# GiannisPikoulis/dsml-thesis

Measured on AMD Instinct MI355X. Metric: DDIM denoise steps/sec (64×64×4 latent, 256² face) at 1/2/4/8 GPUs, higher is better.
Workload: dtype f32; 1 GPU; face_reenactment emotion-conditioned LDM (AffectNet config), DDIM-200 schedule, 16 samples/GPU, 64x64x4 latent, CFG off, eta 0, random-init weights; batch_per_gpu=16, global_batch=16, ddim_steps=200, hipgraph=True

## Files before the change

### dsml_thesis_amd/csrc/winograd.hip

```cpp
#include "ldmk_common.h"
#include "ldmk_split.h"

namespace ldmk {

__global__ __launch_bounds__(256) void wino_input_kernel(const float* __restrict__ x0, int c0, const float* __restrict__ x1,
                                                         int c1, const float* __restrict__ coef, int silu, int H, int W,
                                                         long long tiles, float* __restrict__ V) {
  const int C = c0 + c1, c4n = C >> 2;
  const int tw = W >> 1, th = H >> 1;
  const long long total = tiles * c4n;
  for (long long idx = (long long)blockIdx.x * blockDim.x + threadIdx.x; idx < total; idx += (long long)gridDim.x * blockDim.x) {
    const long long t = idx / c4n;
    const int c = (int)(idx - t * c4n) * 4;
    const int tx = (int)(t % tw);
    const long long t2 = t / tw;
    const int ty = (int)(t2 % th), n = (int)(t2 / th);
    const float* src = c < c0 ? x0 + (long long)n * H * W * c0 + c : x1 + (long long)n * H * W * c1 + (c - c0);
    const int cs = c < c0 ? c0 : c1;
    float4 sc = make_float4(1.f, 1.f, 1.f, 1.f), sh = make_float4(0.f, 0.f, 0.f, 0.f);
    if (coef) {
      const float* cf = coef + ((long long)n * 2) * C + c;
      sc = *reinterpret_cast<const float4*>(cf);
      sh = *reinterpret_cast<const float4*>(cf + C);
    }
// ... 88 lines not shown
    const int cs = c < c0 ? c0 : c1;
    float4 sc[2] = {make_float4(1.f, 1.f, 1.f, 1.f), make_float4(1.f, 1.f, 1.f, 1.f)};
    float4 sh[2] = {make_float4(0.f, 0.f, 0.f, 0.f), make_float4(0.f, 0.f, 0.f, 0.f)};
    if (coef) {
      const float* cf = coef + ((long long)n * 2) * C + c;
      sc[0] = *reinterpret_cast<const float4*>(cf); sc[1] = *reinterpret_cast<const float4*>(cf + 4);
      sh[0] = *reinterpret_cast<const float4*>(cf + C); sh[1] = *reinterpret_cast<const float4*>(cf + C + 4);
    }
#pragma unroll
    for (int i = 0; i < 4; ++i) {
      const int y = 2 * ty - 1 + i;
#pragma unroll
      for (int j = 0; j < 4; ++j) {
        const int x = 2 * tx - 1 + j;
        const bool in = y >= 0 && y < H && x >= 0 && x < W;
#pragma unroll
        for (int e = 0; e < 2; ++e) {
          float4 v = make_float4(0.f, 0.f, 0.f, 0.f);
          if (in) {
            v = *reinterpret_cast<const float4*>(src + ((long long)y * W + x) * cs + 4 * e);
            if (coef) { v.x = fmaf(v.x, sc[e].x, sh[e].x); v.y = fmaf(v.y, sc[e].y, sh[e].y); v.z = fmaf(v.z, sc[e].z, sh[e].z); v.w = fmaf(v.w, sc[e].w, sh[e].w); }
            if (silu) { v.x = silu_f(v.x); v.y = silu_f(v.y); v.z = silu_f(v.z); v.w = silu_f(v.w); }
          }
          d[i][j][e] = v;
        }
      }
    }
  } else {
#pragma unroll
    for (int i = 0; i < 4; ++i)
#pragma unroll
      for (int j = 0; j < 4; ++j) d[i][j][0] = d[i][j][1] = make_float4(0.f, 0.f, 0.f, 0.f);
  }
  auto sub = [](float4 a, float4 b) { return make_float4(a.x - b.x, a.y - b.y, a.z - b.z, a.w - b.w); };
  auto add = [](float4 a, float4 b) { return make_float4(a.x + b.x, a.y + b.y, a.z + b.z, a.w + b.w); };
  unsigned char* dst = V + ((long long)blockIdx.x * Kb + slab) * (PL * 1024) + lane * 16;
#pragma unroll
  for (int i = 0; i < 4; ++i) {
    float4 rr[4][2];
#pragma unroll
    for (int e = 0; e < 2; ++e)
#pragma unroll
      for (int j = 0; j < 4; ++j) {
        rr[j][e] = i == 0 ? sub(d[0][j][e], d[2][j][e]) : i == 1 ? add(d[1][j][e], d[2][j][e]) : i == 2 ? sub(d[2][j][e], d[1][j][e])
                                                                                                          : sub(d[1][j][e], d[3][j][e]);
      }
    wino_store_ps<PL>(dst + (4 * i + 0) * plane_bytes, sub(rr[0][0], rr[2][0]), sub(rr[0][1], rr[2][1]), range_flag);
    wino_store_ps<PL>(dst + (4 * i + 1) * plane_bytes, add(rr[1][0], rr[2][0]), add(rr[1][1], rr[2][1]), range_flag);
    wino_store_ps<PL>(dst + (4 * i + 2) * plane_bytes, sub(rr[2][0], rr[1][0]), sub(rr[2][1], rr[1][1]), range_flag);
    wino_store_ps<PL>(dst + (4 * i + 3) * plane_bytes, sub(rr[1][0], rr[3][0]), sub(rr[1][1], rr[3][1]), range_flag);
  }
}

constexpr int WINO_MAX_CHUNKS = 8;
__global__ __launch_bounds__(256) void wino_output_kernel(const float* __restrict__ Mb, const float* __restrict__ bias,
                                                          const float* __restrict__ bvec, int bvec_ld,
                                                          const float* __restrict__ res, float* __restrict__ out,
                                                          float* __restrict__ stats, int H, int W, int N, int R,
                                                          long long tiles) {
  const int tw = W >> 1, th = H >> 1;
  const int bands = th / R;
  const int n = blockIdx.x / bands, band = blockIdx.x - n * bands;
  const long long ps = tiles * N;
  const int nchunks = (2 * R * W) >> 5;
  const int c = blockIdx.y * blockDim.x + threadIdx.x;
  if (c < N) {
    const float add0 = (bias ? bias[c] : 0.f) + (bvec ? bvec[(long long)n * bvec_ld + c] : 0.f);
    float shift[WINO_MAX_CHUNKS], sm[WINO_MAX_CHUNKS], sq[WINO_MAX_CHUNKS];
    bool have[WINO_MAX_CHUNKS];
#pragma unroll
    for (int k = 0; k < WINO_MAX_CHUNKS; ++k) { shift[k] = 0.f; sm[k] = 0.f; sq[k] = 0.f; have[k] = false; }
    for (int r = 0; r < R; ++r) {
      const int ty = band * R + r;
      for (int tx = 0; tx < tw; ++tx) {
        const long long t = ((long long)n * th + ty) * tw + tx;
        const float* mp = Mb + t * N + c;
        float m[16];
#pragma unroll
        for (int p = 0; p < 16; ++p) m[p] = mp[p * ps];
        float s0[4], s1[4];
#pragma unroll
        for (int j = 0; j < 4; ++j) {
          s0[j] = (m[j] + m[4 + j]) + m[8 + j];
          s1[j] = (m[4 + j] - m[8 + j]) - m[12 + j];
        }
        float y[2][2];
        y[0][0] = (s0[0] + s0[1]) + s0[2];
        y[0][1] = (s0[1] - s0[2]) - s0[3];
        y[1][0] = (s1[0] + s1[1]) + s1[2];
        y[1][1] = (s1[1] - s1[2]) - s1[3];
#pragma unroll
        for (int i = 0; i < 2; ++i)
#pragma unroll
          for (int j = 0; j < 2; ++j) {
            const int yy = 2 * ty + i, xx = 2 * tx + j;
            const long long o = (((long long)n * H + yy) * W + xx) * N + c;
            float v = y[i][j] + add0;
            if (res) v += res[o];
            out[o] = v;
            if (stats) {
              const int k = (((2 * r + i) * W) + xx) >> 5;
#pragma unroll
              for (int q = 0; q < WINO_MAX_CHUNKS; ++q)
                if (q == k) {
                  if (!have[q]) { shift[q] = v; have[q] = true; }
                  const float dv = v - shift[q];
                  sm[q] += dv;
                  sq[q] = fmaf(dv, dv, sq[q]);
                }
            }
          }
      }
    }
    if (stats) {
      const long long chunk0 = ((long long)n * H * W + (long long)band * 2 * R * W) >> 5;
#pragma unroll
      for (int q = 0; q < WINO_MAX_CHUNKS; ++q)
        if (q < nchunks) {
          float* d = stats + ((chunk0 + q) * N + c) * 3;
          d[0] = shift[q]; d[1] = sm[q]; d[2] = sq[q];
        }
    }
  }
}

}

extern "C" long long ldmk_winograd_tiles(int n, int h, int w) { return (long long)n * (h / 2) * (w / 2); }

extern "C" int ldmk_winograd_input(const float* x0, int c0, const float* x1, int c1, const float* coef, int silu, int n, int h,
                                   int w, float* v, void* stream) {
  LDMK_ENTER();
  using namespace ldmk;
  LDMK_REQUIRE(x0 && v && n > 0 && c0 > 0, "ldmk_winograd_input: bad args");
  LDMK_REQUIRE((c1 == 0) == (x1 == nullptr), "ldmk_winograd_input: x1/c1 mismatch");
  LDMK_REQUIRE(h >= 2 && w >= 2 && h % 2 == 0 && w % 2 == 0, "ldmk_winograd_input: H=%d W=%d must be even", h, w);
  LDMK_REQUIRE(c0 % 4 == 0 && c1 % 4 == 0, "ldmk_winograd_input: channel counts must be multiples of 4");
  const long long tiles = ldmk_winograd_tiles(n, h, w);
  const long long total = tiles * ((c0 + c1) / 4);
  long long g = (total + 255) / 256;
  if (g > 16384) g = 16384;
  hipLaunchKernelGGL(wino_input_kernel, dim3((unsigned)g), dim3(256), 0, (hipStream_t)stream, x0, c0, x1, c1, coef, silu, h, w,
                     tiles, v);
  return check_launch("ldmk_winograd_input");
}

extern "C" long long ldmk_ps_bytes(int rows, int k);
extern "C" long long ldmk_ps_bytes_h2(int rows, int k);

static int winograd_input_ps_any(const float* x0, int c0, const float* x1, int c1, const float* coef, int silu, int n, int h, int w, void* v_ps,
                                 int* range_flag, void* stream);

extern "C" int ldmk_winograd_input_ps(const float* x0, int c0, const float* x1, int c1, const float* coef, int silu, int n, int h,
                                      int w, void* v_ps, void* stream) {
  return winograd_input_ps_any(x0, c0, x1, c1, coef, silu, n, h, w, v_ps, nullptr, stream);
}

extern "C" int ldmk_winograd_input_ps_h2(const float* x0, int c0, const float* x1, int c1, const float* coef, int silu, int n, int h,
                                         int w, void* v_ps, int* range_flag, void* stream) {
  LDMK_ENTER();
  LDMK_REQUIRE(range_flag != nullptr, "ldmk_winograd_input_ps_h2: range_flag");
  return winograd_input_ps_any(x0, c0, x1, c1, coef, silu, n, h, w, v_ps, range_flag, stream);
}

static int winograd_input_ps_any(const float* x0, int c0, const float* x1, int c1, const float* coef, int silu, int n, int h, int w, void* v_ps,
                                 int* range_flag, void* stream) {
  LDMK_ENTER();
  using namespace ldmk;
  LDMK_REQUIRE(x0 && v_ps && n > 0 && c0 > 0, "ldmk_winograd_input_ps: bad args");
  LDMK_REQUIRE((c1 == 0) == (x1 == nullptr), "ldmk_winograd_input_ps: x1/c1 mismatch");
  LDMK_REQUIRE(h >= 2 && w >= 2 && h % 2 == 0 && w % 2 == 0, "ldmk_winograd_input_ps: H=%d W=%d must be even", h, w);
  LDMK_REQUIRE(c0 % 16 == 0 && c1 % 16 == 0, "ldmk_winograd_input_ps: channel counts must be multiples of 16 (k-slabs of the PS layout)");
  const long long tiles = ldmk_winograd_tiles(n, h, w);
  LDMK_REQUIRE(tiles < (1LL << 31), "ldmk_winograd_input_ps: too many tiles");
  const int C = c0 + c1;
  const dim3 grid((unsigned)((tiles + 31) / 32), (C / 16 + 3) / 4);
  if (range_flag)
    hipLaunchKernelGGL(wino_input_ps_kernel<2>, grid, dim3(256), 0, (hipStream_t)stream, x0, c0, x1, c1, coef, silu, h, w, tiles,
                       reinterpret_cast<unsigned char*>(v_ps), ldmk_ps_bytes_h2((int)tiles, C), range_flag);
  else
    hipLaunchKernelGGL(wino_input_ps_kernel<3>, grid, dim3(256), 0, (hipStream_t)stream, x0, c0, x1, c1, coef, silu, h, w, tiles,
                       reinterpret_cast<unsigned char*>(v_ps), ldmk_ps_bytes((int)tiles, C), range_flag);
  return check_launch("ldmk_winograd_input_ps");
}

extern "C" int ldmk_winograd_output(const float* m, const float* bias, const float* batch_vec, int batch_vec_ld,
                                    const float* residual, float* out, float* stats_out, int n, int h, int w, int cout,
                                    void* stream) {
  LDMK_ENTER();
  using namespace ldmk;
  LDMK_REQUIRE(m && out && n > 0 && cout > 0, "ldmk_winograd_output: bad args");
  LDMK_REQUIRE(h >= 2 && w >= 2 && h % 2 == 0 && w % 2 == 0, "ldmk_winograd_output: H=%d W=%d must be even", h, w);
  int R = 1;
  if (stats_out) {
    while ((2 * R * w) % 32 != 0 && R < h / 2) R *= 2;
    LDMK_REQUIRE((2 * R * w) % 32 == 0 && (h / 2) % R == 0 && (2 * R * w) / 32 <= WINO_MAX_CHUNKS && (h * w) % 32 == 0,
                 "ldmk_winograd_output: stats_out needs bands of whole 32-pixel chunks (H=%d W=%d)", h, w);
  }
  const long long tiles = ldmk_winograd_tiles(n, h, w);
  hipLaunchKernelGGL(wino_output_kernel, dim3(n * ((h / 2) / R), (cout + 255) / 256), dim3(256), 0, (hipStream_t)stream, m, bias, batch_vec,
                     batch_vec_ld, residual, out, stats_out, h, w, cout, R, tiles);
  return check_launch("ldmk_winograd_output");
}

namespace ldmk {

__global__ __launch_bounds__(256) void upconv_gather_kernel(const float* __restrict__ x, int C, int H, int W, long long pix,
                                                            float* __restrict__ A) {
  const int c4n = C >> 2;
  const long long total = pix * c4n;
  for (long long idx = (long long)blockIdx.x * blockDim.x + threadIdx.x; idx < total; idx += (long long)gridDim.x * blockDim.x) {
    const long long p = idx / c4n;
    const int c = (int)(idx - p * c4n) * 4;
    const int xx = (int)(p % W);
    const long long p2 = p / W;
    const int yy = (int)(p2 % H), n = (int)(p2 / H);
    float4 d[3][3];
#pragma unroll
    for (int i = 0; i < 3; ++i)
#pragma unroll
      for (int j = 0; j < 3; ++j) {
        const int y = yy - 1 + i, x_ = xx - 1 + j;
        d[i][j] = (y >= 0 && y < H && x_ >= 0 && x_ < W)
                      ? *reinterpret_cast<const float4*>(x + (((long long)n * H + y) * W + x_) * C + c)
                      : make_float4(0.f, 0.f, 0.f, 0.f);
      }
    const long long plane = pix * 4 * C;
#pragma unroll
    for (int a = 0; a < 2; ++a)
#pragma unroll
      for (int b = 0; b < 2; ++b) {
        float* dst = A + (long long)(2 * a + b) * plane + p * 4 * C + c;
#pragma unroll
        for (int i = 0; i < 2; ++i)
#pragma unroll
          for (int j = 0; j < 2; ++j) *reinterpret_cast<float4*>(dst + (2 * i + j) * C) = d[a + i][b + j];
      }
  }
}

template <int PL>
__global__ __launch_bounds__(256) void upconv_gather_ps_kernel(const float* __restrict__ x, int C, int H, int W, long long pix,
                                                               unsigned char* __restrict__ A, long long plane_bytes, int* __restrict__ range_flag) {
  const int Kc = C >> 4;
  const int lane = threadIdx.x & 63, wave = threadIdx.x >> 6;
  const int r = lane & 31, hh = lane >> 5;
  const int slab = blockIdx.y * 4 + wave;
  if (slab >= Kc) return;
  const long long p = (long long)blockIdx.x * 32 + r;
  const int c = slab * 16 + hh * 8;
  float4 d[3][3][2];
#pragma unroll
  for (int i = 0; i < 3; ++i)
#pragma unroll
    for (int j = 0; j < 3; ++j) d[i][j][0] = d[i][j][1] = make_float4(0.f, 0.f, 0.f, 0.f);
// ... 133 lines not shown
```

### dsml_thesis_amd/lib.py

```python
import ctypes as C
import os

from . import switches

_HERE = os.path.dirname(os.path.abspath(__file__))
LIB_PATH = switches.get("LDMK_LIBRARY") or os.path.join(_HERE, "libldmk.so")

A_ROWS, A_CONV3X3 = 0, 1
TF_NONE, TF_AFFINE, TF_AFFINE_SILU, TF_LAYERNORM, TF_LAYERNORM_FOLDED = 0, 1, 2, 3, 4
EPI_NONE, EPI_GEGLU = 0, 1
COMPUTE_F32, COMPUTE_BF16, COMPUTE_BF16X3, COMPUTE_F16X2 = 0, 1, 2, 3
POST_NONE, POST_GROUPNORM, POST_LAYERNORM = 0, 1, 2

_fp = C.c_void_p


class IgemmArgs(C.Structure):
    _fields_ = [
        ("M", C.c_int), ("N", C.c_int), ("K", C.c_int),
        ("a0", _fp), ("a1", _fp), ("c0", C.c_int), ("c1", C.c_int),
        ("a_mode", C.c_int), ("in_h", C.c_int), ("in_w", C.c_int), ("out_h", C.c_int), ("out_w", C.c_int),
        ("stride", C.c_int), ("pad_lo", C.c_int), ("upsample", C.c_int),
        ("a_tf", C.c_int), ("tf_coef", _fp), ("row_stats", _fp), ("ln_gamma", _fp), ("ln_beta", _fp),
        ("rows_per_sample", C.c_int),
# ... 11 lines not shown
        ("w_split", _fp), ("w_split_ld", C.c_int), ("w_split_bstride", C.c_longlong),
        ("a_split", _fp), ("a_split_ld", C.c_int),
        ("a_ps", _fp), ("a_ps_bstride", C.c_longlong), ("w_ps", _fp), ("w_ps_bstride", C.c_longlong), ("out_ps", _fp),
        ("w_scale_exp", C.c_int), ("range_flag", _fp),
        ("attn_kv_out", _fp), ("attn_tokens", C.c_int), ("attn_heads", C.c_int),
        ("a_ps1", _fp), ("a_ps_k0", C.c_int),
    ]


class PostArgs(C.Structure):
    _fields_ = [
        ("src", _fp), ("nslab", C.c_int), ("slab_stride", C.c_longlong), ("M", C.c_int), ("N", C.c_int),
        ("rows_per_sample", C.c_int), ("alpha", C.c_float), ("bias", _fp), ("batch_vec", _fp), ("batch_vec_ld", C.c_int),
        ("residual", _fp), ("ldr", C.c_int), ("geglu", C.c_int), ("raw_out", _fp), ("ld_raw", C.c_int), ("norm", C.c_int),
        ("x1", _fp), ("c1", C.c_int), ("groups", C.c_int), ("eps", C.c_float), ("gamma", _fp), ("beta", _fp),
        ("silu", C.c_int), ("norm_out", _fp), ("ld_norm", C.c_int), ("gn_cache_floats", C.c_int),
        ("gn_scratch", _fp), ("gn_scratch_elems", C.c_longlong),
    ]


class WgradArgs(C.Structure):
    _fields_ = [
        ("R", C.c_int), ("Kw", C.c_int), ("N", C.c_int), ("a", _fp), ("c", C.c_int), ("lda", C.c_int),
        ("a_mode", C.c_int), ("in_h", C.c_int), ("in_w", C.c_int), ("out_h", C.c_int), ("out_w", C.c_int),
        ("stride", C.c_int), ("pad_lo", C.c_int), ("upsample", C.c_int),
        ("dy", _fp), ("ldy", C.c_int), ("dw", _fp), ("ldw", C.c_int), ("accumulate", C.c_int), ("alpha", C.c_float),
        ("batch", C.c_int), ("a_bstride", C.c_longlong), ("dy_bstride", C.c_longlong), ("dw_bstride", C.c_longlong),
        ("splitr", C.c_int), ("ws", _fp), ("ws_elems", C.c_longlong), ("dbias", _fp), ("compute", C.c_int),
    ]


_SIGS = {
    "ldmk_version": (C.c_int, []),
    "ldmk_last_error": (C.c_char_p, []),
    "ldmk_init": (C.c_int, [C.c_int]),
    "ldmk_igemm": (C.c_int, [C.POINTER(IgemmArgs), _fp]),
    "ldmk_igemm_workspace_elems": (C.c_longlong, [C.POINTER(IgemmArgs)]),
    "ldmk_igemm_check": (C.c_int, [C.POINTER(IgemmArgs)]),
    "ldmk_igemm_plan": (C.c_int, [C.POINTER(IgemmArgs), C.POINTER(C.c_int), C.POINTER(C.c_int)]),
    "ldmk_igemm_force_config": (None, [C.c_int]),
    "ldmk_wfrag_elems": (C.c_longlong, [C.c_int, C.c_int]),
    "ldmk_pack_wfrag": (C.c_int, [_fp, C.c_int, C.c_int, C.c_int, _fp, _fp]),
    "ldmk_pack_wsplit": (C.c_int, [_fp, C.c_int, C.c_int, C.c_int, C.c_int, C.c_longlong, _fp, C.c_int, _fp]),
    "ldmk_pack_wsplit_h2": (C.c_int, [_fp, C.c_int, C.c_int, C.c_int, C.c_int, C.c_longlong, C.c_int, _fp, C.c_int, _fp]),
    "ldmk_pack_wbf16t": (C.c_int, [_fp, C.c_int, C.c_int, C.c_int, _fp, C.c_int, _fp]),
    "ldmk_winograd_tiles": (C.c_longlong, [C.c_int, C.c_int, C.c_int]),
    "ldmk_winograd_input": (C.c_int, [_fp, C.c_int, _fp, C.c_int, _fp, C.c_int, C.c_int, C.c_int, C.c_int, _fp, _fp]),
    "ldmk_winograd_input_ps": (C.c_int, [_fp, C.c_int, _fp, C.c_int, _fp, C.c_int, C.c_int, C.c_int, C.c_int, _fp, _fp]),
    "ldmk_winograd_output": (C.c_int, [_fp, _fp, _fp, C.c_int, _fp, _fp, _fp, C.c_int, C.c_int, C.c_int, C.c_int, _fp]),
    "ldmk_upconv_gather": (C.c_int, [_fp, C.c_int, C.c_int, C.c_int, C.c_int, _fp, _fp]),
    "ldmk_upconv_gather_ps": (C.c_int, [_fp, C.c_int, C.c_int, C.c_int, C.c_int, _fp, _fp]),
    "ldmk_upconv_gather_ps_h2": (C.c_int, [_fp, C.c_int, C.c_int, C.c_int, C.c_int, _fp, _fp, _fp]),
    "ldmk_winograd_input_ps_h2": (C.c_int, [_fp, C.c_int, _fp, C.c_int, _fp, C.c_int, C.c_int, C.c_int, C.c_int, _fp, _fp, _fp]),
    "ldmk_upconv_scatter": (C.c_int, [_fp, _fp, _fp, _fp, C.c_int, C.c_int, C.c_int, C.c_int, _fp]),
    "ldmk_fold_layernorm": (C.c_int, [_fp, C.c_int, C.c_int, C.c_int, _fp, _fp, _fp, _fp, _fp, _fp, _fp]),
    "ldmk_attn_force_qt": (None, [C.c_int]),
    "ldmk_gn_chunks": (C.c_int, [C.c_int]),
    "ldmk_gn_partial": (C.c_int, [_fp, C.c_int, C.c_int, C.c_int, _fp, _fp]),
    "ldmk_gn_finalize": (C.c_int, [_fp, C.c_int, _fp, C.c_int, C.c_int, C.c_int, C.c_int, C.c_float, _fp, _fp, _fp, _fp]),
    "ldmk_gn_coef": (C.c_int, [_fp, C.c_int, _fp, C.c_int, C.c_int, C.c_int, C.c_int, C.c_float, _fp, _fp, _fp, _fp, _fp]),
    "ldmk_ln_stats": (C.c_int, [_fp, C.c_int, C.c_int, C.c_float, _fp, _fp]),
    "ldmk_ln_stats_guard": (C.c_int, [_fp, C.c_int, C.c_int, C.c_float, _fp, C.c_float, _fp, _fp]),
    "ldmk_ps_bytes": (C.c_longlong, [C.c_int, C.c_int]),
    "ldmk_pack_ps": (C.c_int, [_fp, C.c_int, C.c_int, C.c_longlong, C.c_longlong, C.c_int, C.c_longlong, _fp, _fp]),
    "ldmk_ps_bytes_h2": (C.c_longlong, [C.c_int, C.c_int]),
    "ldmk_pack_ps_h2": (C.c_int, [_fp, C.c_int, C.c_int, C.c_longlong, C.c_longlong, C.c_int, C.c_longlong, C.c_int, _fp, _fp, _fp]),
    "ldmk_ln_stats_ps_h2": (C.c_int, [_fp, C.c_int, C.c_int, C.c_float, _fp, _fp, C.c_float, _fp, _fp, _fp]),
    "ldmk_ln_stats_ps": (C.c_int, [_fp, C.c_int, C.c_int, C.c_float, _fp, _fp, C.c_float, _fp, _fp]),
    "ldmk_ln_stats_split": (C.c_int, [_fp, C.c_int, C.c_int, C.c_float, _fp, _fp, C.c_int, _fp]),
    "ldmk_gn_apply": (C.c_int, [_fp, C.c_int, _fp, C.c_int, _fp, _fp, C.c_int, C.c_int, C.c_int, _fp]),
    "ldmk_gn_coef_film": (C.c_int, [_fp, _fp, C.c_int, C.c_int, C.c_int, _fp]),
    "ldmk_gn_apply_ps_h2": (C.c_int, [_fp, C.c_int, _fp, C.c_int, _fp, _fp, C.c_int, C.c_int, C.c_int, _fp, _fp]),
    "ldmk_post": (C.c_int, [C.POINTER(PostArgs), _fp]),
    "ldmk_post_scratch_elems": (C.c_longlong, [C.POINTER(PostArgs)]),
    "ldmk_attn_self": (C.c_int, [_fp, _fp, C.c_int, C.c_int, C.c_int, C.c_float, _fp]),
    "ldmk_attn_self_x3": (C.c_int, [_fp, _fp, C.c_int, C.c_int, C.c_int, C.c_float, _fp]),
    "ldmk_attn_kv_split_bytes": (C.c_longlong, [C.c_int, C.c_int, C.c_int]),
    "ldmk_attn_self_x3p": (C.c_int, [_fp, _fp, _fp, C.c_int, C.c_int, C.c_int, C.c_float, _fp]),
    "ldmk_attn_self_x3p_ps": (C.c_int, [_fp, _fp, _fp, _fp, C.c_int, C.c_int, C.c_int, C.c_float, _fp]),
    "ldmk_attn_kv_split_h2_bytes": (C.c_longlong, [C.c_int, C.c_int, C.c_int]),
    "ldmk_attn_self_h2": (C.c_int, [_fp, _fp, _fp, _fp, C.c_int, C.c_int, C.c_int, C.c_float, _fp]),
    "ldmk_attn_self_h2_ps": (C.c_int, [_fp, _fp, _fp, _fp, _fp, C.c_int, C.c_int, C.c_int, C.c_float, _fp]),
    "ldmk_attn_self_h2_tiles": (C.c_int, [_fp, _fp, _fp, _fp, _fp, C.c_int, C.c_int, C.c_int, C.c_float, _fp]),
    "ldmk_attn_self_small": (C.c_int, [_fp, C.c_int, C.c_longlong, _fp, C.c_int, C.c_int, C.c_int, C.c_float, _fp]),
    "ldmk_attn_cross": (C.c_int, [_fp, C.c_int, _fp, _fp, C.c_int, _fp, C.c_int, C.c_int, C.c_int, C.c_int, C.c_int,
                                  C.c_float, _fp]),
    "ldmk_attn_cross_d": (C.c_int, [_fp, C.c_int, _fp, _fp, C.c_int, _fp, C.c_int, C.c_int, C.c_int, C.c_int, C.c_int, C.c_int, C.c_float, _fp]),
    "ldmk_heads_gather": (C.c_int, [_fp, C.c_int, C.c_int, _fp, C.c_int, C.c_int, C.c_int, C.c_int, C.c_int, _fp]),
    "ldmk_heads_scatter": (C.c_int, [_fp, _fp, C.c_int, C.c_int, C.c_int, C.c_int, C.c_int, C.c_int, _fp]),
    "ldmk_softmax_rows": (C.c_int, [_fp, C.c_longlong, C.c_int, C.c_float, _fp]),
    "ldmk_dense_small": (C.c_int, [_fp, C.c_int, _fp, _fp, _fp, C.c_int, C.c_int, C.c_int, C.c_int, C.c_int, _fp]),
    "ldmk_timestep_embedding": (C.c_int, [_fp, _fp, _fp, C.c_int, C.c_int, _fp]),
    "ldmk_conv3x3_in": (C.c_int, [_fp, C.c_int, _fp, C.c_int, _fp, _fp, _fp, C.c_int, C.c_int, C.c_int, C.c_int, _fp]),
    "ldmk_conv3x3_out": (C.c_int, [_fp, _fp, _fp, _fp, _fp, C.c_int, C.c_int, C.c_int, C.c_int, C.c_int, _fp]),
    "ldmk_conv3x3_out_small": (C.c_int, [_fp, _fp, _fp, _fp, _fp, C.c_int, C.c_int, C.c_int, C.c_int, C.c_int, _fp]),
    "ldmk_conv1x1_nchw": (C.c_int, [_fp, _fp, _fp, _fp, C.c_int, C.c_int, C.c_int, C.c_int, _fp]),
    "ldmk_ddim_step": (C.c_int, [_fp, _fp, _fp, _fp, _fp, C.c_float, C.c_int, _fp, _fp, C.c_longlong, C.c_int, _fp, _fp,
                                 C.c_int, C.c_int, C.c_int, _fp]),
    "ldmk_advance_timestep": (C.c_int, [_fp, _fp, _fp, C.c_int, C.c_int, C.c_int, _fp]),
    "ldmk_ddpm_step": (C.c_int, [_fp, _fp, _fp, _fp, _fp, _fp, _fp, C.c_longlong, C.c_int, _fp]),
    "ldmk_vq_nearest": (C.c_int, [_fp, _fp, _fp, _fp, C.c_int, C.c_int, C.c_int, C.c_int, _fp]),
    "ldmk_permute3": (C.c_int, [_fp, _fp, C.c_int, C.c_int, C.c_int, C.c_int, C.c_int, C.c_int, _fp]),
    "ldmk_audio_attention": (C.c_int, [_fp, C.c_int, C.c_int, C.c_int, _fp, _fp, _fp, _fp, _fp, _fp]),
    "ldmk_mask_rows": (C.c_int, [_fp, _fp, C.c_int, C.c_int, C.c_int, C.c_int, C.c_float, _fp]),
    "ldmk_pack_conv3x3": (C.c_int, [_fp, _fp, C.c_int, C.c_int, _fp]),
    "ldmk_postprocess_frames": (C.c_int, [_fp, _fp, C.c_int, C.c_int, C.c_int, _fp]),
# ... 100 lines not shown
```

### dsml_thesis_amd/switches.py

```python
import os

SWITCHES = {
    "LDMK_SPLIT_BF16": ("1", "arithmetic", "0: every GEMM and the attention on the f32 matrix-core form (v_mfma_f32_32x32x2_f32); the "
                        "f32_mfma_form leg of bench.py"),
    "LDMK_F16X2": ("1", "arithmetic", "0: split products from the exact bf16x3 split (six bf16 MFMAs, operands bit-exact) instead of "
                   "F16X2 (three fp16 MFMAs, range-checked per site); the bf16x3_form leg of bench.py"),
    "LDMK_LN_UNFOLDED": (None, "arithmetic", "set: LayerNorm applied in the GEMM prologue instead of folded through the product (what "
                         "the folded-LayerNorm guard switches a model to by itself)"),
    "LDMK_LN_GUARD_RATIO": ("4.0", "arithmetic", "|mean| / std of a token row above which the folded LayerNorm raises its guard"),
    "LDMK_ATTN_H2_MIN_TOKENS": ("512", "arithmetic", "self attention runs in F16X2 from this many tokens per sample, bf16x3 below"),
    "LDMK_H2_CONV_RULE": ("1", "arithmetic", "0: untabled long-K convolutions (K >= 1440) do not take the F16X2 rule"),
    "LDMK_PS": ("1", "route", "0: no pre-split (PS layout, LDS-DMA) GEMM tiles; same bits"),
    "LDMK_PSC": ("1", "route", "0: no conv-mode pre-split tile for 3x3 convolutions; same bits"),
    "LDMK_PSC_FORCE": (None, "route", "'cfg,splitk': force the conv-mode pre-split tile for every eligible convolution (A/B runs)"),
    "LDMK_POUT_PS": ("0", "route", "1: SpatialTransformer.proj_out on a pre-split tile instead of the row GEMM (measured slower)"),
    "LDMK_FOLD_POUT": ("1", "route", "0: the last block's ff.net.2 and proj_out stay two GEMMs instead of one pre-split GEMM on two A "
                       "sources with the composed weight (other bits, same tolerance)"),
    "LDMK_ATTN_PS": ("1", "route", "0: attn1.to_out does not read the attention result in the PS layout"),
    "LDMK_ATTN_PRESPLIT": ("1", "route", "0: K / V are split inside the attention kernel instead of once by their producer; same bits"),
    "LDMK_ATTN_PRESPLIT_MIN_TOKENS": ("2048", "route", "tokens per sample from which K / V are pre-split"),
    "LDMK_QKV_TILES": ("1", "route", "0: the fused QKV projection does not write the attention's K / V tiles from its epilogue"),
    "LDMK_NO_WINOGRAD": (None, "route", "set: no Winograd F(2x2,3x3) convolutions and no phase-split upsampling convolutions (direct "
                         "implicit GEMM everywhere; other bits, same tolerance)"),
    "LDMK_WINO_MIN_TILES": ("256", "route", "Winograd from this many 2x2 output tiles at the plan-policy batch"),
    "LDMK_WINO_MIN_CIN": ("320", "route", "Winograd / phase-split upsampling from this many input channels"),
    "LDMK_NO_SMALL_ROUTE": (None, "route", "set: batch 1-2 jobs run the batched launch program instead of the small-batch route"),
    "LDMK_SMALL_ROWS": ("4096", "route", "rows (batch x pixels at the policy batch) up to which the small-batch route is taken"),
    "LDMK_SPLITK_IN_LAUNCH": (None, "route", "set: split-K slabs combined by each tile's last workgroup instead of a reduce launch "
                              "(measured slower)"),
    "LDMK_TRAIN_NO_PACKED_W": (None, "route", "set: the training step's bf16 GEMMs read fp32 weights instead of the packed bf16 copies"),
    "LDMK_ATTN_QT": (None, "route", "1 | 2: query tiles per wave of the staged f32 attention kernel (A/B hook)"),
    "LDMK_NO_PLAN_TABLE": (None, "plan", "set: ignore igemm_plans.json (the library's built-in tile heuristic plans every GEMM)"),
    "LDMK_PLAN_MAX_RATIO": ("0", "plan", "> 0: a tuned plan is used only within this ratio of its tuned row count (0: nearest at any "
                            "distance)"),
    "LDMK_PLAN_TABLE": (None, "plan", "a file that replaces the `f32` section of igemm_plans.json (a flat {key: [cfg, splitk]} file as "
                        "the tuning tools write it, or another merged file whose section is taken)"),
    "LDMK_X3_TABLE": (None, "plan", "the same for the `bf16x3` section"),
    "LDMK_H2_TABLE": (None, "plan", "the same for the `f16x2` section"),
    "LDMK_PS_TABLE": (None, "plan", "the same for the `ps_bf16x3` section (pre-split tiles)"),
    "LDMK_PS_H2_TABLE": (None, "plan", "the same for the `ps_f16x2` section (pre-split tiles, F16X2)"),
    "LDMK_LIBRARY": (None, "runtime", "path of the libldmk.so to load instead of the in-tree one"),
    "LDMK_FORCE_COLLECTIVE": (None, "runtime", "set: parallel.all_gather_items issues the real all-gather at world size 1 too (RCCL "
                              "rehearsal; bench.py sets it under LDMK_BENCH_FORCE_DIST)"),
    "LDMK_LIB_OUT": (None, "build", "output path of the build (an A/B build next to the shipped library)"),
    "LDMK_HIPCC_FLAGS": ("", "build", "extra hipcc flags, part of the build digest (-DLDMK_PS_PROBES, -DLDMK_IG_STAMPS: probe builds "
                         "for tools/; the shipped library carries neither)"),
    "LDMK_ATTN_QB": (None, "library", "1 | 2: 32-query blocks per wave of the pre-split attention kernels (default by token count); "
                     "same bits"),
    "LDMK_ATTN_XCD": ("1", "library", "0: F16X2 attention workgroups in launch order instead of re-dealt over the XCDs; same bits"),
    "LDMK_ATTN_PIPE": ("2", "library", "F16X2 attention key loop: 2 pipelined + lazy running maximum, 1 pipelined with the exact "
                       "maximum, 0 phase-separated (1 and 0: same bits)"),
    "LDMK_IG_NFAST": ("1", "library", "0: LDS-tiled igemm workgroups in row-major tile order instead of column tiles adjacent; same bits"),
    "LDMK_IG_LEAN": ("1", "library", "0: the general igemm epilogue everywhere instead of the operand-set specialised copies; same bits"),
    "LDMK_PS_NFAST": ("1", "library", "as LDMK_IG_NFAST, pre-split tiles"),
    "LDMK_PS_LEAN": ("1", "library", "as LDMK_IG_LEAN, pre-split tiles"),
    "LDMK_WGRAD_TR": ("1", "library", "0: bf16 weight-gradient GEMM with the strided gather instead of transposed LDS reads (A/B)"),
    "LDMK_BENCH_BACKEND": ("nccl", "bench", "'gloo': rehearse the N > 1 path of bench.py on a one-GPU box"),
    "LDMK_BENCH_FORCE_DIST": (None, "bench", "set: create the process group and issue the clip leg's collective with a single rank"),
}

PROBE_ONLY = ("LDMK_PS_DEBUG", "LDMK_PS_STAGGER")


def get(name, default=None):
    if name not in SWITCHES:
        raise KeyError(f"{name} is not a registered switch (dsml_thesis_amd/switches.py)")
    return os.environ.get(name, default)


def table_markdown():
    rows = ["| switch | default | scope | effect |", "|---|---|---|---|"]
    for name, (default, scope, doc) in SWITCHES.items():
        shown = "unset" if default is None else ("`" + (default or "''") + "`")
        rows.append(f"| `{name}` | {shown} | {scope} | {doc} |")
    return "\n".join(rows)


if __name__ == "__main__":
    print(table_markdown())
```

### include/ldmk.h

```cpp
#ifndef LDMK_H
#define LDMK_H
#ifdef __cplusplus
extern "C" {
#endif

#define LDMK_OK 0
#define LDMK_EINVAL (-1)
#define LDMK_EHIP (-2)
#define LDMK_ENOMEM (-3)

int ldmk_version(void);
const char* ldmk_last_error(void);
int ldmk_init(int device);

enum { LDMK_A_ROWS = 0, LDMK_A_CONV3X3 = 1 };
enum { LDMK_TF_NONE = 0, LDMK_TF_AFFINE = 1, LDMK_TF_AFFINE_SILU = 2, LDMK_TF_LAYERNORM = 3,
       LDMK_TF_LAYERNORM_FOLDED = 4 };
enum { LDMK_EPI_NONE = 0, LDMK_EPI_GEGLU = 1 };
enum { LDMK_COMPUTE_F32 = 0, LDMK_COMPUTE_BF16 = 1, LDMK_COMPUTE_BF16X3 = 2, LDMK_COMPUTE_F16X2 = 3 };
#define LDMK_F16X2_A_EXP 6
#define LDMK_F16X2_RANGE 1000.0f

typedef struct ldmk_igemm_args {
  int M, N, K;
// ... 42 lines not shown
  long long w_split_bstride;
  const void* a_split;
  int a_split_ld;
  const void* a_ps;
  long long a_ps_bstride;
  const void* w_ps;
  long long w_ps_bstride;
  void* out_ps;
  int w_scale_exp;
  int* range_flag;
  void* attn_kv_out;
  int attn_tokens;
  int attn_heads;
  const void* a_ps1;
  int a_ps_k0;
} ldmk_igemm_args;

long long ldmk_ps_bytes(int rows, int k);
int ldmk_pack_ps(const float* src, int rows, int k, long long row_stride, long long k_stride, int batch, long long src_bstride,
                 void* dst, void* stream);
int ldmk_ln_stats_ps(const float* x, int rows, int c, float eps, float* stats, void* dst, float guard, int* flag, void* stream);

long long ldmk_ps_bytes_h2(int rows, int k);
int ldmk_pack_ps_h2(const float* src, int rows, int k, long long row_stride, long long k_stride, int batch, long long src_bstride,
                    int scale_exp, int* range_flag, void* dst, void* stream);
int ldmk_ln_stats_ps_h2(const float* x, int rows, int c, float eps, float* stats, void* dst, float guard, int* flag, int* range_flag,
                        void* stream);
int ldmk_gn_apply_ps_h2(const float* x0, int c0, const float* x1, int c1, const float* coef, void* y_ps, int n, int hw, int silu,
                        int* range_flag, void* stream);

int ldmk_pack_wsplit(const float* w, int K, int N, int ldb, int batch, long long w_bstride, void* out, int ld_out, void* stream);
int ldmk_pack_wsplit_h2(const float* w, int K, int N, int ldb, int batch, long long w_bstride, int scale_exp, void* out, int ld_out,
                        void* stream);
int ldmk_pack_wbf16t(const float* w, int K, int N, int ldb, void* out, int ld_out, void* stream);

int ldmk_igemm(const ldmk_igemm_args* args, void* stream);
long long ldmk_igemm_workspace_elems(const ldmk_igemm_args* args);
int ldmk_igemm_check(const ldmk_igemm_args* args);
long long ldmk_wfrag_elems(int K, int N);
int ldmk_pack_wfrag(const float* w, int ldb, int K, int N, float* wfrag, void* stream);
int ldmk_fold_layernorm(const float* w, int ldb, int K, int N, const float* gamma, const float* beta, const float* bias,
                        float* w_out, float* colsum, float* bias_out, void* stream);
int ldmk_igemm_plan(const ldmk_igemm_args* args, int* tile_cfg, int* splitk);

long long ldmk_winograd_tiles(int n, int h, int w);
int ldmk_winograd_input(const float* x0, int c0, const float* x1, int c1, const float* coef, int silu, int n, int h, int w,
                        float* v, void* stream);
int ldmk_winograd_input_ps(const float* x0, int c0, const float* x1, int c1, const float* coef, int silu, int n, int h, int w,
                           void* v_ps, void* stream);
int ldmk_winograd_input_ps_h2(const float* x0, int c0, const float* x1, int c1, const float* coef, int silu, int n, int h, int w,
                              void* v_ps, int* range_flag, void* stream);
int ldmk_winograd_output(const float* m, const float* bias, const float* batch_vec, int batch_vec_ld, const float* residual,
                         float* out, float* stats_out, int n, int h, int w, int cout, void* stream);

int ldmk_upconv_gather(const float* x, int c, int n, int h, int w, float* a, void* stream);
int ldmk_upconv_gather_ps(const float* x, int c, int n, int h, int w, void* a_ps, void* stream);
int ldmk_upconv_gather_ps_h2(const float* x, int c, int n, int h, int w, void* a_ps, int* range_flag, void* stream);
int ldmk_upconv_scatter(const float* planes, const float* bias, float* out, float* stats_out, int n, int h, int w, int cout,
                        void* stream);

int ldmk_gn_chunks(int hw);
int ldmk_gn_partial(const float* x, int c, int n, int hw, float* partial, void* stream);
int ldmk_gn_finalize(const float* partial0, int c0, const float* partial1, int c1, int n, int hw, int groups,
                     float eps, const float* gamma, const float* beta, float* coef, void* stream);
int ldmk_gn_coef(const float* x0, int c0, const float* x1, int c1, int n, int hw, int groups, float eps,
                 const float* gamma, const float* beta, float* partial, float* coef, void* stream);
int ldmk_ln_stats(const float* x, int rows, int c, float eps, float* stats, void* stream);
int ldmk_ln_stats_guard(const float* x, int rows, int c, float eps, float* stats, float guard, int* flag, void* stream);
int ldmk_ln_stats_split(const float* x, int rows, int C, float eps, float* stats, void* split, int ld_split, void* stream);
int ldmk_gn_apply(const float* x0, int c0, const float* x1, int c1, const float* coef, float* y, int n, int hw,
                  int silu, void* stream);
int ldmk_resample2(const float* x, float* y, int n, int h, int w, int c, int up, void* stream);
int ldmk_gn_coef_film(float* coef, const float* emb, int ld, int n, int c, void* stream);

enum { LDMK_POST_NONE = 0, LDMK_POST_GROUPNORM = 1, LDMK_POST_LAYERNORM = 2 };
typedef struct ldmk_post_args {
  const float* src;
  int nslab;
  long long slab_stride;
  int M, N;
  int rows_per_sample;
  float alpha;
  const float* bias;
  const float* batch_vec;
  int batch_vec_ld;
  const float* residual;
  int ldr;
  int geglu;
  float* raw_out;
  int ld_raw;
  int norm;
  const float* x1;
  int c1;
  int groups;
  float eps;
  const float* gamma;
  const float* beta;
  int silu;
  float* norm_out;
  int ld_norm;
  int gn_cache_floats;
  float* gn_scratch;
  long long gn_scratch_elems;
} ldmk_post_args;
#define LDMK_POST_GN_TILED_ROWS 512
int ldmk_post(const ldmk_post_args* args, void* stream);
// ... 152 lines not shown
```

Measured before the change: 1142 sample-steps/s.

## Stage Winograd input patches in LDS and vectorise the output transform

```diff
diff --git a/dsml_thesis_amd/csrc/winograd.hip b/dsml_thesis_amd/csrc/winograd.hip
--- a/dsml_thesis_amd/csrc/winograd.hip
+++ b/dsml_thesis_amd/csrc/winograd.hip
@@ -164,6 +164,71 @@
   }
 }
 
+struct WinoStageGeom { int S, RS, PR, PC; };
+
+template <int PL>
+__global__ __launch_bounds__(256) void wino_input_ps_staged_kernel(const float* __restrict__ x0, int c0, const float* __restrict__ x1,
+                                                                   int c1, const float* __restrict__ coef, int silu, int H, int W,
+                                                                   int NS, unsigned char* __restrict__ V, long long plane_bytes,
+                                                                   int* __restrict__ range_flag, WinoStageGeom g) {
+  extern __shared__ float4 wino_patch4[];
+  float* patch = reinterpret_cast<float*>(wino_patch4);
+  constexpr int Q = 4, PST = 16 + 4;
+  const int C = c0 + c1, Kb = C >> 4;
+  const int tw = W >> 1, th = H >> 1;
+  const int slab = blockIdx.y;
+  {
+    const long long t0 = (long long)blockIdx.x * 32;
+    const int tx0 = (int)(t0 % tw);
+    const long long g0 = t0 / tw;
+    const int ty0 = (int)(g0 % th), n0 = (int)(g0 / th);
+    const int y0 = 2 * ty0 - 1, xo = 2 * tx0 - 1;
+    const int items = g.S * g.PR * g.PC * Q;
+    for (int it = threadIdx.x; it < items; it += 256) {
+      const int q = it % Q, px = it / Q;
+      const int pc = px % g.PC, prs = px / g.PC;
+      const int pr = prs % g.PR, n = n0 + prs / g.PR;
+      const int y = y0 + pr, x = xo + pc, c = slab * 16 + 4 * q;
+      float4 v = make_float4(0.f, 0.f, 0.f, 0.f);
+      if (n < NS && y >= 0 && y < H && x >= 0 && x < W) {
+        const float* src = c < c0 ? x0 + (((long long)n * H + y) * W + x) * c0 + c : x1 + (((long long)n * H + y) * W + x) * c1 + (c - c0);
+        v = *reinterpret_cast<const float4*>(src);
+        if (coef) {
+          const float* cf = coef + ((long long)n * 2) * C + c;
+          const float4 sc = *reinterpret_cast<const float4*>(cf), sh = *reinterpret_cast<const float4*>(cf + C);
+          v.x = fmaf(v.x, sc.x, sh.x); v.y = fmaf(v.y, sc.y, sh.y); v.z = fmaf(v.z, sc.z, sh.z); v.w = fmaf(v.w, sc.w, sh.w);
+        }
+        if (silu) { v.x = silu_f(v.x); v.y = silu_f(v.y); v.z = silu_f(v.z); v.w = silu_f(v.w); }
+      }
+      *reinterpret_cast<float4*>(patch + px * PST + 4 * q) = v;
+    }
+  }
+  __syncthreads();
+  const int lane = threadIdx.x & 63, wave = threadIdx.x >> 6;
+  const int r = lane & 31, hh = lane >> 5;
+  const int i = wave;
+  const int k = tw >= 32 ? 0 : r / tw, txl = tw >= 32 ? r : r % tw;
+  const int row = (k / g.RS) * g.PR + 2 * (k % g.RS), col = 2 * txl;
+  const int ra = i == 0 ? 0 : i == 2 ? 2 : 1, rb = i == 0 ? 2 : i == 1 ? 2 : i == 2 ? 1 : 3;
+  const float* pa = patch + ((row + ra) * g.PC + col) * PST + hh * 8;
+  const float* pb = patch + ((row + rb) * g.PC + col) * PST + hh * 8;
+  auto sub = [](float4 a, float4 b) { return make_float4(a.x - b.x, a.y - b.y, a.z - b.z, a.w - b.w); };
+  auto add = [](float4 a, float4 b) { return make_float4(a.x + b.x, a.y + b.y, a.z + b.z, a.w + b.w); };
+  float4 rr[4][2];
+#pragma unroll
+  for (int j = 0; j < 4; ++j)
+#pragma unroll
+    for (int e = 0; e < 2; ++e) {
+      const float4 da = *reinterpret_cast<const float4*>(pa + j * PST + 4 * e), db = *reinterpret_cast<const float4*>(pb + j * PST + 4 * e);
+      rr[j][e] = i == 1 ? add(da, db) : sub(da, db);
+    }
+  unsigned char* dst = V + ((long long)blockIdx.x * Kb + slab) * (PL * 1024) + lane * 16;
+  wino_store_ps<PL>(dst + (4 * i + 0) * plane_bytes, sub(rr[0][0], rr[2][0]), sub(rr[0][1], rr[2][1]), range_flag);
+  wino_store_ps<PL>(dst + (4 * i + 1) * plane_bytes, add(rr[1][0], rr[2][0]), add(rr[1][1], rr[2][1]), range_flag);
+  wino_store_ps<PL>(dst + (4 * i + 2) * plane_bytes, sub(rr[2][0], rr[1][0]), sub(rr[2][1], rr[1][1]), range_flag);
+  wino_store_ps<PL>(dst + (4 * i + 3) * plane_bytes, sub(rr[1][0], rr[3][0]), sub(rr[1][1], rr[3][1]), range_flag);
+}
+
 constexpr int WINO_MAX_CHUNKS = 8;
 __global__ __launch_bounds__(256) void wino_output_kernel(const float* __restrict__ Mb, const float* __restrict__ bias,
                                                           const float* __restrict__ bvec, int bvec_ld,
@@ -236,6 +301,95 @@
   }
 }
 
+constexpr int WINO_OUT_CB = 64;
+__global__ __launch_bounds__(256) void wino_output_vec_kernel(const float* __restrict__ Mb, const float* __restrict__ bias,
+                                                              const float* __restrict__ bvec, int bvec_ld,
+                                                              const float* __restrict__ res, float* __restrict__ out,
+                                                              float* __restrict__ stats, int H, int W, int N, int R, long long tiles) {
+  extern __shared__ float4 wino_band4[];
+  float* bandv = reinterpret_cast<float*>(wino_band4);
+  const int tw = W >> 1, th = H >> 1;
+  const int bands = th / R;
+  const int n = blockIdx.x / bands, band = blockIdx.x - n * bands;
+  const long long ps = tiles * N;
+  const int cb = blockIdx.y * WINO_OUT_CB;
+  {
+    const int q = threadIdx.x & 15, c = cb + 4 * q;
+    if (c < N) {
+      float add0[4];
+#pragma unroll
+      for (int e = 0; e < 4; ++e) add0[e] = (bias ? bias[c + e] : 0.f) + (bvec ? bvec[(long long)n * bvec_ld + c + e] : 0.f);
+      for (int tl = threadIdx.x >> 4; tl < R * tw; tl += blockDim.x >> 4) {
+        const int r = tl / tw, tx = tl - r * tw;
+        const int ty = band * R + r;
+        const long long t = ((long long)n * th + ty) * tw + tx;
+        const float* mp = Mb + t * N + c;
+        float4 m4[16];
+#pragma unroll
+        for (int p = 0; p < 16; ++p) m4[p] = *reinterpret_cast<const float4*>(mp + p * ps);
+        float y[2][2][4];
+#pragma unroll
+        for (int e = 0; e < 4; ++e) {
+          float m[16];
+#pragma unroll
+          for (int p = 0; p < 16; ++p) m[p] = e == 0 ? m4[p].x : e == 1 ? m4[p].y : e == 2 ? m4[p].z : m4[p].w;
+          float s0[4], s1[4];
+#pragma unroll
+          for (int j = 0; j < 4; ++j) {
+            s0[j] = (m[j] + m[4 + j]) + m[8 + j];
+            s1[j] = (m[4 + j] - m[8 + j]) - m[12 + j];
+          }
+          y[0][0][e] = (s0[0] + s0[1]) + s0[2];
+          y[0][1][e] = (s0[1] - s0[2]) - s0[3];
+          y[1][0][e] = (s1[0] + s1[1]) + s1[2];
+          y[1][1][e] = (s1[1] - s1[2]) - s1[3];
+        }
+#pragma unroll
+        for (int i = 0; i < 2; ++i)
+#pragma unroll
+          for (int j = 0; j < 2; ++j) {
+            const int yy = 2 * ty + i, xx = 2 * tx + j;
+            const long long o = (((long long)n * H + yy) * W + xx) * N + c;
+            float4 v = make_float4(y[i][j][0] + add0[0], y[i][j][1] + add0[1], y[i][j][2] + add0[2], y[i][j][3] + add0[3]);
+            if (res) {
+              const float4 rv = *reinterpret_cast<const float4*>(res + o);
+              v.x += rv.x; v.y += rv.y; v.z += rv.z; v.w += rv.w;
+            }
+            *reinterpret_cast<float4*>(out + o) = v;
+            if (stats) *reinterpret_cast<float4*>(bandv + ((2 * r + i) * W + xx) * WINO_OUT_CB + 4 * q) = v;
+          }
+      }
+    }
+  }
+  if (!stats) return;
+  __syncthreads();
+  const int cl = threadIdx.x & 63, c = cb + cl;
+  const int nchunks = (2 * R * W) >> 5;
+  if (c >= N) return;
+  const long long chunk0 = ((long long)n * H * W + (long long)band * 2 * R * W) >> 5;
+  for (int k = threadIdx.x >> 6; k < nchunks; k += blockDim.x >> 6) {
+    float shift = 0.f, sm = 0.f, sq = 0.f;
+    bool have = false;
+    for (int r = 0; r < R; ++r)
+      for (int tx = 0; tx < tw; ++tx)
+#pragma unroll
+        for (int i = 0; i < 2; ++i)
+#pragma unroll
+          for (int j = 0; j < 2; ++j) {
+            const int pi = (2 * r + i) * W + 2 * tx + j;
+            if ((pi >> 5) == k) {
+              const float v = bandv[pi * WINO_OUT_CB + cl];
+              if (!have) { shift = v; have = true; }
+              const float dv = v - shift;
+              sm += dv;
+              sq = fmaf(dv, dv, sq);
+            }
+          }
+    float* d = stats + ((chunk0 + k) * N + c) * 3;
+    d[0] = shift; d[1] = sm; d[2] = sq;
+  }
+}
+
 }
 
 extern "C" long long ldmk_winograd_tiles(int n, int h, int w) { return (long long)n * (h / 2) * (w / 2); }
@@ -260,23 +414,81 @@
 extern "C" long long ldmk_ps_bytes(int rows, int k);
 extern "C" long long ldmk_ps_bytes_h2(int rows, int k);
 
+static int wino_staged_env() {
+  static const int v = [] { const char* e = getenv("LDMK_WINO_STAGED"); return e ? atoi(e) : 1; }();
+  return v;
+}
+
+static bool wino_stage_geom(int h, int w, ldmk::WinoStageGeom* g) {
+  const int tw = w / 2, th = h / 2;
+  if (tw >= 32 && tw % 32 == 0) {
+    *g = {1, 1, 4, 66};
+    return true;
+  }
+  if (tw < 4 || 32 % tw != 0) return false;
+  const int R = 32 / tw;
+  if (th % R == 0) *g = {1, R, 2 * R + 2, w + 2};
+  else if (R % th == 0) *g = {R / th, th, 2 * th + 2, w + 2};
+  else return false;
+  return true;
+}
+
+extern "C" int ldmk_winograd_input_ps_route(int n, int h, int w, int c0, int c1) {
+  ldmk::WinoStageGeom g;
+  if (n <= 0 || h < 2 || w < 2 || h % 2 || w % 2 || c0 <= 0 || c0 % 16 || c1 < 0 || c1 % 16) return 0;
+  return wino_stage_geom(h, w, &g) ? 1 : 0;
+}
+
+extern "C" int ldmk_winograd_output_route(int n, int h, int w, int cout, int with_stats) {
+  if (n <= 0 || h < 2 || w < 2 || h % 2 || w % 2 || cout <= 0 || cout % 4) return 0;
+  if (with_stats) {
+    int R = 1;
+    while ((2 * R * w) % 32 != 0 && R < h / 2) R *= 2;
+    if (2 * R * w > 128) return 0;
+  }
+  return 1;
+}
+
 static int winograd_input_ps_any(const float* x0, int c0, const float* x1, int c1, const float* coef, int silu, int n, int h, int w, void* v_ps,
-                                 int* range_flag, void* stream);
+                                 int* range_flag, bool staged, void* stream);
 
 extern "C" int ldmk_winograd_input_ps(const float* x0, int c0, const float* x1, int c1, const float* coef, int silu, int n, int h,
                                       int w, void* v_ps, void* stream) {
-  return winograd_input_ps_any(x0, c0, x1, c1, coef, silu, n, h, w, v_ps, nullptr, stream);
+  return winograd_input_ps_any(x0, c0, x1, c1, coef, silu, n, h, w, v_ps, nullptr, wino_staged_env() != 0, stream);
+}
+
+extern "C" int ldmk_winograd_input_ps_v1(const float* x0, int c0, const float* x1, int c1, const float* coef, int silu, int n, int h,
+                                         int w, void* v_ps, void* stream) {
+  return winograd_input_ps_any(x0, c0, x1, c1, coef, silu, n, h, w, v_ps, nullptr, false, stream);
 }
 
 extern "C" int ldmk_winograd_input_ps_h2(const float* x0, int c0, const float* x1, int c1, const float* coef, int silu, int n, int h,
                                          int w, void* v_ps, int* range_flag, void* stream) {
   LDMK_ENTER();
   LDMK_REQUIRE(range_flag != nullptr, "ldmk_winograd_input_ps_h2: range_flag");
-  return winograd_input_ps_any(x0, c0, x1, c1, coef, silu, n, h, w, v_ps, range_flag, stream);
+  return winograd_input_ps_any(x0, c0, x1, c1, coef, silu, n, h, w, v_ps, range_flag, wino_staged_env() != 0, stream);
+}
+
+extern "C" int ldmk_winograd_input_ps_h2_v1(const float* x0, int c0, const float* x1, int c1, const float* coef, int silu, int n, int h,
+                                            int w, void* v_ps, int* range_flag, void* stream) {
+  LDMK_ENTER();
+  LDMK_REQUIRE(range_flag != nullptr, "ldmk_winograd_input_ps_h2: range_flag");
+  return winograd_input_ps_any(x0, c0, x1, c1, coef, silu, n, h, w, v_ps, range_flag, false, stream);
+}
+
+template <int PL>
+static void wino_input_ps_staged_launch(const float* x0, int c0, const float* x1, int c1, const float* coef, int silu, int n, int h, int w,
+                                        long long tiles, void* v_ps, long long plane_bytes, int* range_flag, const ldmk::WinoStageGeom& g,
+                                        void* stream) {
+  const int Kb = (c0 + c1) / 16;
+  const dim3 grid((unsigned)((tiles + 31) / 32), Kb);
+  const size_t lds = (size_t)g.S * g.PR * g.PC * (16 + 4) * sizeof(float);
+  hipLaunchKernelGGL(ldmk::wino_input_ps_staged_kernel<PL>, grid, dim3(256), lds, (hipStream_t)stream, x0, c0, x1, c1, coef, silu,
+                     h, w, n, reinterpret_cast<unsigned char*>(v_ps), plane_bytes, range_flag, g);
 }
 
 static int winograd_input_ps_any(const float* x0, int c0, const float* x1, int c1, const float* coef, int silu, int n, int h, int w, void* v_ps,
-                                 int* range_flag, void* stream) {
+                                 int* range_flag, bool staged, void* stream) {
   LDMK_ENTER();
   using namespace ldmk;
   LDMK_REQUIRE(x0 && v_ps && n > 0 && c0 > 0, "ldmk_winograd_input_ps: bad args");
@@ -286,19 +498,25 @@
   const long long tiles = ldmk_winograd_tiles(n, h, w);
   LDMK_REQUIRE(tiles < (1LL << 31), "ldmk_winograd_input_ps: too many tiles");
   const int C = c0 + c1;
+  const long long plane_bytes = range_flag ? ldmk_ps_bytes_h2((int)tiles, C) : ldmk_ps_bytes((int)tiles, C);
+  WinoStageGeom g;
+  if (staged && ldmk_winograd_input_ps_route(n, h, w, c0, c1) && wino_stage_geom(h, w, &g)) {
+    if (range_flag) wino_input_ps_staged_launch<2>(x0, c0, x1, c1, coef, silu, n, h, w, tiles, v_ps, plane_bytes, range_flag, g, stream);
+    else wino_input_ps_staged_launch<3>(x0, c0, x1, c1, coef, silu, n, h, w, tiles, v_ps, plane_bytes, range_flag, g, stream);
+    return check_launch("ldmk_winograd_input_ps");
+  }
   const dim3 grid((unsigned)((tiles + 31) / 32), (C / 16 + 3) / 4);
   if (range_flag)
     hipLaunchKernelGGL(wino_input_ps_kernel<2>, grid, dim3(256), 0, (hipStream_t)stream, x0, c0, x1, c1, coef, silu, h, w, tiles,
-                       reinterpret_cast<unsigned char*>(v_ps), ldmk_ps_bytes_h2((int)tiles, C), range_flag);
+                       reinterpret_cast<unsigned char*>(v_ps), plane_bytes, range_flag);
   else
     hipLaunchKernelGGL(wino_input_ps_kernel<3>, grid, dim3(256), 0, (hipStream_t)stream, x0, c0, x1, c1, coef, silu, h, w, tiles,
-                       reinterpret_cast<unsigned char*>(v_ps), ldmk_ps_bytes((int)tiles, C), range_flag);
+                       reinterpret_cast<unsigned char*>(v_ps), plane_bytes, range_flag);
   return check_launch("ldmk_winograd_input_ps");
 }
 
-extern "C" int ldmk_winograd_output(const float* m, const float* bias, const float* batch_vec, int batch_vec_ld,
-                                    const float* residual, float* out, float* stats_out, int n, int h, int w, int cout,
-                                    void* stream) {
+static int winograd_output_any(const float* m, const float* bias, const float* batch_vec, int batch_vec_ld, const float* residual, float* out,
+                               float* stats_out, int n, int h, int w, int cout, bool vec, void* stream) {
   LDMK_ENTER();
   using namespace ldmk;
   LDMK_REQUIRE(m && out && n > 0 && cout > 0, "ldmk_winograd_output: bad args");
@@ -310,9 +528,30 @@
                  "ldmk_winograd_output: stats_out needs bands of whole 32-pixel chunks (H=%d W=%d)", h, w);
   }
   const long long tiles = ldmk_winograd_tiles(n, h, w);
+  const bool aligned = (((uintptr_t)m | (uintptr_t)out | (uintptr_t)residual) & 15) == 0;
+  if (vec && aligned && ldmk_winograd_output_route(n, h, w, cout, stats_out != nullptr)) {
+    const int band_tiles = R * (w / 2);
+    const int threads = band_tiles * 16 >= 256 ? 256 : band_tiles * 16 <= 64 ? 64 : (band_tiles * 16 + 63) / 64 * 64;
+    const size_t lds = stats_out ? (size_t)2 * R * w * WINO_OUT_CB * sizeof(float) : 0;
+    hipLaunchKernelGGL(wino_output_vec_kernel, dim3(n * ((h / 2) / R), (cout + WINO_OUT_CB - 1) / WINO_OUT_CB), dim3(threads), lds,
+                       (hipStream_t)stream, m, bias, batch_vec, batch_vec_ld, residual, out, stats_out, h, w, cout, R, tiles);
+    return check_launch("ldmk_winograd_output");
+  }
   hipLaunchKernelGGL(wino_output_kernel, dim3(n * ((h / 2) / R), (cout + 255) / 256), dim3(256), 0, (hipStream_t)stream, m, bias, batch_vec,
                      batch_vec_ld, residual, out, stats_out, h, w, cout, R, tiles);
   return check_launch("ldmk_winograd_output");
+}
+
+extern "C" int ldmk_winograd_output(const float* m, const float* bias, const float* batch_vec, int batch_vec_ld,
+                                    const float* residual, float* out, float* stats_out, int n, int h, int w, int cout,
+                                    void* stream) {
+  return winograd_output_any(m, bias, batch_vec, batch_vec_ld, residual, out, stats_out, n, h, w, cout, wino_staged_env() != 0, stream);
+}
+
+extern "C" int ldmk_winograd_output_v1(const float* m, const float* bias, const float* batch_vec, int batch_vec_ld,
+                                       const float* residual, float* out, float* stats_out, int n, int h, int w, int cout,
+                                       void* stream) {
+  return winograd_output_any(m, bias, batch_vec, batch_vec_ld, residual, out, stats_out, n, h, w, cout, false, stream);
 }
 
 namespace ldmk {
diff --git a/dsml_thesis_amd/lib.py b/dsml_thesis_amd/lib.py
--- a/dsml_thesis_amd/lib.py
+++ b/dsml_thesis_amd/lib.py
@@ -87,6 +87,11 @@
     "ldmk_upconv_gather_ps": (C.c_int, [_fp, C.c_int, C.c_int, C.c_int, C.c_int, _fp, _fp]),
     "ldmk_upconv_gather_ps_h2": (C.c_int, [_fp, C.c_int, C.c_int, C.c_int, C.c_int, _fp, _fp, _fp]),
     "ldmk_winograd_input_ps_h2": (C.c_int, [_fp, C.c_int, _fp, C.c_int, _fp, C.c_int, C.c_int, C.c_int, C.c_int, _fp, _fp, _fp]),
+    "ldmk_winograd_input_ps_v1": (C.c_int, [_fp, C.c_int, _fp, C.c_int, _fp, C.c_int, C.c_int, C.c_int, C.c_int, _fp, _fp]),
+    "ldmk_winograd_input_ps_h2_v1": (C.c_int, [_fp, C.c_int, _fp, C.c_int, _fp, C.c_int, C.c_int, C.c_int, C.c_int, _fp, _fp, _fp]),
+    "ldmk_winograd_output_v1": (C.c_int, [_fp, _fp, _fp, C.c_int, _fp, _fp, _fp, C.c_int, C.c_int, C.c_int, C.c_int, _fp]),
+    "ldmk_winograd_input_ps_route": (C.c_int, [C.c_int, C.c_int, C.c_int, C.c_int, C.c_int]),
+    "ldmk_winograd_output_route": (C.c_int, [C.c_int, C.c_int, C.c_int, C.c_int, C.c_int]),
     "ldmk_upconv_scatter": (C.c_int, [_fp, _fp, _fp, _fp, C.c_int, C.c_int, C.c_int, C.c_int, _fp]),
     "ldmk_fold_layernorm": (C.c_int, [_fp, C.c_int, C.c_int, C.c_int, _fp, _fp, _fp, _fp, _fp, _fp, _fp]),
     "ldmk_attn_force_qt": (None, [C.c_int]),
diff --git a/dsml_thesis_amd/switches.py b/dsml_thesis_amd/switches.py
--- a/dsml_thesis_amd/switches.py
+++ b/dsml_thesis_amd/switches.py
@@ -54,6 +54,8 @@
     "LDMK_IG_LEAN": ("1", "library", "0: the general igemm epilogue everywhere instead of the operand-set specialised copies; same bits"),
     "LDMK_PS_NFAST": ("1", "library", "as LDMK_IG_NFAST, pre-split tiles"),
     "LDMK_PS_LEAN": ("1", "library", "as LDMK_IG_LEAN, pre-split tiles"),
+    "LDMK_WINO_STAGED": ("1", "library", "0: the Winograd input / output transforms on their first kernels (a thread loads its own 4x4 "
+                         "window / walks a band's tiles) instead of the LDS-staged / vectorised ones; same bits"),
     "LDMK_WGRAD_TR": ("1", "library", "0: bf16 weight-gradient GEMM with the strided gather instead of transposed LDS reads (A/B)"),
     "LDMK_BENCH_BACKEND": ("nccl", "bench", "'gloo': rehearse the N > 1 path of bench.py on a one-GPU box"),
     "LDMK_BENCH_FORCE_DIST": (None, "bench", "set: create the process group and issue the clip leg's collective with a single rank"),
diff --git a/include/ldmk.h b/include/ldmk.h
--- a/include/ldmk.h
+++ b/include/ldmk.h
@@ -118,6 +118,14 @@
                               void* v_ps, int* range_flag, void* stream);
 int ldmk_winograd_output(const float* m, const float* bias, const float* batch_vec, int batch_vec_ld, const float* residual,
                          float* out, float* stats_out, int n, int h, int w, int cout, void* stream);
+int ldmk_winograd_input_ps_route(int n, int h, int w, int c0, int c1);
+int ldmk_winograd_output_route(int n, int h, int w, int cout, int with_stats);
+int ldmk_winograd_input_ps_v1(const float* x0, int c0, const float* x1, int c1, const float* coef, int silu, int n, int h, int w,
+                              void* v_ps, void* stream);
+int ldmk_winograd_input_ps_h2_v1(const float* x0, int c0, const float* x1, int c1, const float* coef, int silu, int n, int h, int w,
+                                 void* v_ps, int* range_flag, void* stream);
+int ldmk_winograd_output_v1(const float* m, const float* bias, const float* batch_vec, int batch_vec_ld, const float* residual,
+                            float* out, float* stats_out, int n, int h, int w, int cout, void* stream);
 
 int ldmk_upconv_gather(const float* x, int c, int n, int h, int w, float* a, void* stream);
 int ldmk_upconv_gather_ps(const float* x, int c, int n, int h, int w, void* a_ps, void* stream);
```

Result: faster. 1163 sample-steps/s, median of 6 (+1.8%).
